# JiaxuanYou/graph-pooling

Hardware: AMD Instinct MI355X
Metric: graphs/sec fwd+bwd, DD padded batch N_max=500 (higher is better)
Workload: dtype f32; 1 GPU; S-DD: DD-shaped padded batch, B=20/GPU, N_max=500, F=89, H=E=20, K=50, L=3, 1 pool; graphs_per_gpu=20, global_batch=20, linkpred=False, hip_graph=True, parallelism=dp1

## Files before the change

graph_pooling_amd/csrc/dp_common.h:

```cpp
#pragma once
#include <hip/hip_runtime.h>
#include <cstddef>
#include <cstdint>
#include <cstdio>
#include <cstring>
#include <atomic>
#include <mutex>

#include "../../include/diffpool_hip.h"

namespace dp {

void set_error(const char* fmt, ...);
const char* last_error();

#define DP_CHECK_ARG(cond, ...)                      \
    do {                                             \
        if (!(cond)) {                               \
            ::dp::set_error(__VA_ARGS__);            \
            return DP_ERR_INVALID_ARG;               \
        }                                            \
    } while (0)

int* device_error_word();
int* level0_verdict_block();
int device_error_take(bool clear);
int device_error_gate(const char* entry);
#ifdef __HIPCC__
__device__ inline void dev_err_raise(int* word, int bit) {
    if (word) __hip_atomic_fetch_or(word, bit, __ATOMIC_RELAXED, __HIP_MEMORY_SCOPE_SYSTEM);
}

typedef unsigned int u32x4 __attribute__((ext_vector_type(4)));
struct ScBuf {
    __amdgpu_buffer_rsrc_t r;
};
__device__ __forceinline__ ScBuf sc_buf(const void* p, size_t bytes) {
    return ScBuf{__builtin_amdgcn_make_buffer_rsrc(const_cast<void*>(p), 0, (int)bytes, 0x00020000)};
}
__device__ __forceinline__ u32x4 sc_ld16(ScBuf b, unsigned off) { return __builtin_amdgcn_raw_buffer_load_b128(b.r, off, 0, 16); }
__device__ __forceinline__ void sc_st16(ScBuf b, unsigned off, u32x4 v) { __builtin_amdgcn_raw_buffer_store_b128(v, b.r, off, 0, 16); }
__device__ __forceinline__ float sc_ldf(ScBuf b, unsigned off) {
    return __uint_as_float(__builtin_amdgcn_raw_buffer_load_b32(b.r, off, 0, 16));
}
__device__ __forceinline__ void sc_stf(ScBuf b, unsigned off, float v) {
    __builtin_amdgcn_raw_buffer_store_b32(__float_as_uint(v), b.r, off, 0, 16);
}
__device__ __forceinline__ u32x4 sc_tagged(float v0, float v1, unsigned tag) {
    return (u32x4){__float_as_uint(v0), tag, __float_as_uint(v1), tag};
}
#endif

#ifdef __HIPCC__
__device__ __forceinline__ void lds_barrier() {
    asm volatile("" ::: "memory");
    __builtin_amdgcn_s_waitcnt(0xc07f);
    __builtin_amdgcn_s_barrier();
    asm volatile("" ::: "memory");
}
#endif

#ifdef __HIPCC__
template <int CTRL, int ROW_MASK, bool BOUND>
__device__ __forceinline__ float dpp_src(float old, float v) {
    return __int_as_float(__builtin_amdgcn_update_dpp(__float_as_int(old), __float_as_int(v), CTRL, ROW_MASK, 0xF, BOUND));
}
__device__ __forceinline__ float row16_sum(float v) {
    v += dpp_src<0xB1, 0xF, true>(0.f, v);
    v += dpp_src<0x4E, 0xF, true>(0.f, v);
    v += dpp_src<0x141, 0xF, true>(0.f, v);
    v += dpp_src<0x140, 0xF, true>(0.f, v);
    return v;
}
__device__ __forceinline__ float quad4_sum(float v) {
    v += dpp_src<0xB1, 0xF, true>(0.f, v);
    v += dpp_src<0x4E, 0xF, true>(0.f, v);
    return v;
}
__device__ __forceinline__ float oct8_sum(float v) {
    v = quad4_sum(v);
    v += dpp_src<0x141, 0xF, true>(0.f, v);
    return v;
}
__device__ __forceinline__ float row16_max(float v) {
    v = fmaxf(v, dpp_src<0xB1, 0xF, true>(v, v));
    v = fmaxf(v, dpp_src<0x4E, 0xF, true>(v, v));
    v = fmaxf(v, dpp_src<0x141, 0xF, true>(v, v));
    v = fmaxf(v, dpp_src<0x140, 0xF, true>(v, v));
    return v;
}
__device__ __forceinline__ float wave64_sum(float v) {
    v = row16_sum(v);
    v += dpp_src<0x142, 0xA, false>(0.f, v);
    v += dpp_src<0x143, 0xC, false>(0.f, v);
    return __int_as_float(__builtin_amdgcn_readlane(__float_as_int(v), 63));
}
__device__ __forceinline__ float wave64_max(float v) {
    v = row16_max(v);
    v = fmaxf(v, dpp_src<0x142, 0xA, false>(v, v));
    v = fmaxf(v, dpp_src<0x143, 0xC, false>(v, v));
    return __int_as_float(__builtin_amdgcn_readlane(__float_as_int(v), 63));
}
#endif

struct Seq {
    hipStream_t stream;
    char* ws;
    size_t ws_bytes;
    size_t ws_off;
    int err;
    bool dry;
    const int* pred = nullptr;
    void* fold_zero_p = nullptr;
    int fold_zero_n16 = 0;
    int* seq_word = nullptr;

    Seq(hipStream_t s, void* w, size_t wb) : stream(s), ws((char*)w), ws_bytes(wb), ws_off(0), err(0), dry(false) {}
    static Seq sizing() {
        Seq q(nullptr, nullptr, ~size_t(0) >> 1);
        q.dry = true;
        return q;
    }

    template <typename T>
    T* alloc(size_t n) {
        size_t bytes = (n * sizeof(T) + 255) & ~size_t(255);
        if (ws_off + bytes > ws_bytes) {
            if (!err) {
                set_error("workspace too small: need >= %zu bytes, have %zu", ws_off + bytes, ws_bytes);
                err = DP_ERR_WORKSPACE;
            }
            return nullptr;
        }
        T* p = (T*)(ws + ws_off);
        ws_off += bytes;
        return p;
    }
    bool ok() const { return err == 0 && !dry; }
    void copy(void* dst, const void* src, size_t bytes) {
        if (err || dry || bytes == 0) return;
        hipError_t e = hipMemcpyAsync(dst, src, bytes, hipMemcpyDeviceToDevice, stream);
        if (e != hipSuccess) {
            set_error("hipMemcpyAsync: %s", hipGetErrorString(e));
            err = (int)e;
        }
    }
    void check_launch(const char* what) {
        if (err) return;
        hipError_t e = hipGetLastError();
        if (e != hipSuccess) {
            set_error("%s: %s", what, hipGetErrorString(e));
            err = (int)e;
        }
    }
};

inline size_t align256(size_t b) { return (b + 255) & ~size_t(255); }

struct Knobs {
    int agg_wide;
    int agg_rt;
    int agg_debug;
    bool no_pack;
    bool gemm_trace;
    long gemm_target_wgs;
    int node_ksplit;
    bool no_head_fusion;
    bool no_level_fusion;
    bool no_head_fold;
    bool no_split_gemm;
    bool split_gemm_w4;
    bool no_row_quads;
    bool no_rowpart_hook;
    bool no_widen_fusion;
    bool no_agg_first;
    bool no_l0_persist_bwd;
    bool no_l0_persist;
    bool test_barrier_fail;
};
const Knobs& knobs();

struct DynLdsOnce {
    std::atomic<unsigned long long> done{0};
    std::mutex m;
};
void ensure_dyn_lds(Seq& q, DynLdsOnce& st, const void* fn, int bytes, const char* what);

void bgemm(Seq& q, const float* A, const float* B, float* C, const float* bias, int batch, int M, int N,
           int K, int lda, int ldb, int ldc, long sA, long sB, long sC, bool tA, bool tB, float alpha,
           float beta, int act);

#define GEMM_GROUP_MAX 4
struct GemmDesc {
    const float* A;
    const float* B;
    float* C;
    const float* bias;
    int M, N, K;
    int lda, ldb, ldc;
    long sA, sB, sC;
    bool tA, tB;
    float alpha, beta;
    int act;
    long sK;
    int atomic;
    unsigned short* split_out;
    int split_ct, split_k8, split_c0;
    int nosplit;
    float* fix_part;
    int* fix_cnt;
    const float* rp_xhat;
    int rp_ldx;
    float* rp_part;
    int rp_G, rp_g;
};
inline bool gemm_rowpart_ok(int N) { return N >= 1 && N <= 32; }
inline size_t gemm_fix_counters(int batch, int M, int N) {
    return (size_t)batch * ((M + 15) / 16) * ((N + 15) / 16);
}

__device__ inline void bf16_split3(float v, unsigned short& h, unsigned short& m, unsigned short& l) {
    auto rn = [](float x) -> unsigned {
        unsigned u = __float_as_uint(x);
        u += 0x7FFFu + ((u >> 16) & 1u);
        return u >> 16;
    };
    const unsigned hh = rn(v);
    const float r1 = v - __uint_as_float(hh << 16);
    const unsigned mm = rn(r1);
    const float r2 = r1 - __uint_as_float(mm << 16);
    h = (unsigned short)hh;
    m = (unsigned short)mm;
    l = (unsigned short)rn(r2);
}
__device__ __host__ inline long vs_index(int plane, int CTt, int K8, int cb, int k8, int c, int j) {
    return ((((long)plane * CTt + cb) * K8 + k8) * 16 + c) * 8 + j;
}
void bgemm_group(Seq& q, const GemmDesc* d, int count, int batch, int ksplit = 1);
struct GemmPick {
    int bm, bn;
    int ranges[GEMM_GROUP_MAX];
};
GemmPick gemm_pick(const GemmDesc* d, int count, int batch, int ksplit, bool hooked, long target);
long gemm_target_wgs();
int bgemm_plan(const GemmDesc* d, int count, int batch, int ksplit, int* plan_out);
bool gemm_split_usable(const GemmDesc& d, int batch, int ksplit);
void gemm_split_bf16(Seq& q, const GemmDesc& d, int batch);

struct RowGroups {
    int G;
    int c0[2];
    int w[2];
};
struct GroupPtrs {
    float* p[2];
    int ld[2];
};
struct GroupCPtrs {
    const float* p[2];
    int ld[2];
};

struct RowPick {
    int kernel;
    int nk;
    int quad;
    int finalize;
    int zero;
    bool generic() const { return kernel == DP_ROWK_SOFTMAX_FWD || kernel == DP_ROWK_SOFTMAX_BWD; }
};
RowPick rownorm_fwd_pick(const RowGroups& g);
RowPick rownorm_bwd_pick(const RowGroups& g, bool has_bn, int Bs);
RowPick bn_apply_fwd_pick(const RowGroups& g, bool has_part, int Bs);
RowPick softmax_mask_fwd_pick(int K, bool vs, bool zero, bool zero_aligned);
RowPick softmax_mask_bwd_pick(int K, bool dbias);
RowPick masked_max_fwd_pick(int n);
void rownorm_fwd(Seq& q, const float* U, int ldu, const float* P , GroupCPtrs bias,
                 RowGroups g, GroupPtrs yout, float* invn, float* part , long rows,
                 int normalize, int relu_stats);
void bn_apply_fwd(Seq& q, const float* Y, int ldy, const float* part , float* stats,
                  RowGroups g, GroupPtrs xout, int B, int n, int relu, int Bs = 0);
bool bn_transform_supported(RowGroups gin, RowGroups gout, int B);
void bn_transform_fwd(Seq& q, const float* Y, int ldy, const float* part, float* stats, RowGroups gin, GroupPtrs xout,
                      const float* const W[2], RowGroups gout, float* P, int ldp, int B, int n, int relu,
                      unsigned short* vs );
void mask_rows(Seq& q, const float* src, int lds, float* dst, int ldd, const int* num_nodes, int B, int n, int F);
void bn_bwd_partials(Seq& q, GroupCPtrs dx, GroupCPtrs xhat, RowGroups g, float* part, long rows);
void rownorm_bwd(Seq& q, GroupCPtrs dx, GroupCPtrs xhat , GroupCPtrs y,
                 const float* invn, const float* stats, const float* part2, RowGroups g, float* dU, int ldu,
                 const GroupPtrs* dbias , int B, int n, int has_relu, int has_bn,
                 int normalize, unsigned short* vs = nullptr ,
                 int Bs = 0 );
int rownorm_bwd_chunks(int n);
void colsum_batched(Seq& q, const float* X, int ldx, long strideX, int rows, int cols, float* out,
                    long strideOut, int batch, int rowsplit = 1, bool add = false );
void softmax_mask_fwd(Seq& q, const float* logits, int ldl, float* S, int lds, const int* num_nodes, int B,
                      int n, int K, float* S2 = nullptr, unsigned short* vs = nullptr, void* zero_p = nullptr,
                      size_t zero_bytes = 0);
void softmax_mask_bwd(Seq& q, const float* S, int lds, const float* dS, int ldds, const int* num_nodes,
                      float* dlogits, int ldl, int B, int n, int K, float* dbias = nullptr, long dbias_stride = 0,
                      const float* dS2 = nullptr );
void masked_max_fwd(Seq& q, const float* Z, int ldz, const int* num_nodes, float* out, int ldo, int* argmax,
                    int lda, int B, int n, int F);
void masked_max_bwd(Seq& q, const float* dout, int ldo, const int* argmax, int lda, float* dZ, int ldz, int B,
                    int n, int F);
void relu_bwd_inplace(Seq& q, float* d, const float* h, long count);
void argmax_rows(Seq& q, const float* X, int ldx, long long* out, int rows, int cols);
void ce_fwd(Seq& q, const float* logits, const long long* label, float* loss, float* prob, int B, int C,
            float* also_zero = nullptr ,
            float* dunit = nullptr );
void ce_bwd(Seq& q, const float* prob, const long long* label, const float* dloss, float scale, float* dlogits,
            int B, int C);
void reduce_slabs(Seq& q, const float* slabs, long stride, int B, float* out, long count, int accumulate);
void axpy(Seq& q, float* y, const float* x, float a, long count);
void mask_mul(Seq& q, const float* x, int ldx, const float* m, float* out, long rows, int w);
void mask_axpy(Seq& q, float* dst, int ldd, const float* src, const float* m, long rows, int w);
bool rownorm_bwd_mv_supported(RowGroups g, const int din[2], int n);
void rownorm_bwd_mv(Seq& q, GroupCPtrs dx, GroupCPtrs xhat, GroupCPtrs y, const float* invn, const float* stats,
                    const float* part2, RowGroups g, float* dU, int ldu, const GroupPtrs* dbias, int B, int n,
                    int has_relu, int has_bn, int normalize, int Bs, const float* const W[2], const int din[2],
                    const int c0in[2], float* dUin, int lddu);
bool widen_fwd_supported(RowGroups g, const int din[2]);
void widen_fwd(Seq& q, const float* Uin, int ldin, const int c0in[2], const int din[2], const float* const W[2],
               GroupCPtrs bias, RowGroups g, GroupPtrs yout, float* invn, long rows, int normalize);
void gather_cols(Seq& q, const float* x0, int ld0, int w0, const float* x1, int ld1, int w1, float* out, long rows);
bool scatter_add_cols_part_supported(int w0, int w1);
void scatter_add_cols_part(Seq& q, const float* src, GroupPtrs d, GroupCPtrs xhat, int w0, int w1, int G, float* part,
                           long rows);
void scatter_add_cols(Seq& q, const float* src, float* d0, int ld0, int w0, float* d1, int ld1, int w1, long rows);
void zero_fill(Seq& q, void* p, size_t bytes);
void zero_small(Seq& q, void* p, size_t bytes);

struct PackedAdj {
    const unsigned short* A;
    const unsigned short* At;
    int ld;
    const int* flag;
};
void adj_pack(Seq& q, const float* A, unsigned short* P, unsigned short* Pt, int* flag, int B, int n, int ld,
              bool flag_zeroed = false, void* zero_p = nullptr, size_t zero_bytes = 0);
int adj_pack_ld(int n);
bool adj_pack_supported(int n, int C);
size_t split3_elems(int B, int n, int C);
void aggregate(Seq& q, const float* A, const float* V, int ldv, float* U, int ldu, int B, int n, int C, bool trans,
               float beta, const PackedAdj* pk = nullptr, unsigned short* vs = nullptr, bool vs_ready = false);
bool aggregate_rownorm_fwd(Seq& q, const float* A, const float* V, int ldv, const float* P, GroupCPtrs bias,
                           RowGroups g, GroupPtrs yout, float* invn, float* part, int B, int n, int normalize,
                           int stats_mode, const PackedAdj* pk = nullptr, unsigned short* vs = nullptr,
                           bool vs_ready = false);
bool aggregate_packed_usable(const float* A, int n, int C);
struct AggPick {
    int form;
    int ct;
    int rt;
    int tiles, grid;
    size_t lds;
    int fallback;
    int fb_ct, fb_rt, fb_tiles, fb_grid;
    size_t fb_lds;
    bool packed;
    bool declines;
// ... 227 lines not shown
```

graph_pooling_amd/csrc/dp_head.hip:

```cpp
#include "dp_common.h"

namespace dp {

#ifdef DP_STAMP
__device__ unsigned long long g_head_stamps[16];
#define HEAD_STAMP(i)                                                                                 \
    do {                                                                                              \
        if (blockIdx.x == 0 && threadIdx.x == 0) g_head_stamps[i] = __builtin_amdgcn_s_memtime();     \
    } while (0)
#else
#define HEAD_STAMP(i) \
    do {              \
    } while (0)
#endif

constexpr int HEAD_FWD_LDS_FLOATS = 30 * 1024;
constexpr int HEAD_BWD_LDS_FLOATS = 38 * 1024;

__device__ inline float head_wave_sum(float v) {
    return wave64_sum(v);
}

template <int NT>
__device__ inline void head_stage(float* dst, const float* src, int cnt) {
    for (int e0 = 0; e0 < cnt; e0 += NT * 16) {
        float t[16];
#pragma unroll
        for (int u = 0; u < 16; ++u) t[u] = src[min(e0 + u * NT + (int)threadIdx.x, cnt - 1)];
#pragma unroll
        for (int u = 0; u < 16; ++u) {
            const int i = e0 + u * NT + (int)threadIdx.x;
            if (i < cnt) dst[i] = t[u];
        }
    }
}

template <int NT, typename Idx>
__device__ __forceinline__ void stage_issue(float (&t)[16], const float* src, int cnt, int e0, Idx idx) {
#pragma unroll
    for (int u = 0; u < 16; ++u) {
        if (e0 + u * NT >= cnt) break;
        t[u] = src[idx(min(e0 + u * NT + (int)threadIdx.x, cnt - 1))];
    }
}
template <int NT>
__device__ __forceinline__ void stage_commit(float* dst, const float (&t)[16], int cnt, int e0) {
#pragma unroll
    for (int u = 0; u < 16; ++u) {
        if (e0 + u * NT >= cnt) break;
        const int i = e0 + u * NT + (int)threadIdx.x;
        if (i < cnt) dst[i] = t[u];
    }
}
template <int NT, typename Idx>
__device__ inline void stage_rest(float* dst, const float* src, int cnt, Idx idx) {
    for (int e0 = NT * 16; e0 < cnt; e0 += NT * 16) {
        float t[16];
        stage_issue<NT>(t, src, cnt, e0, idx);
        stage_commit<NT>(dst, t, cnt, e0);
    }
}

struct HeadSizes {
    int wtot, btot, mx, hsum;
};
__host__ __device__ inline HeadSizes head_sizes(const HeadArgs& a) {
    HeadSizes z{0, 0, 0, 0};
    for (int i = 0; i < a.n_pred; ++i) {
        z.wtot += a.dims[i] * a.dims[i + 1];
        z.btot += a.dims[i + 1];
    }
    for (int i = 0; i <= a.n_pred; ++i) {
        z.mx = a.dims[i] > z.mx ? a.dims[i] : z.mx;
        z.hsum += a.dims[i];
    }
    return z;
}


__global__ __launch_bounds__(256) void k_head_fwd(HeadArgs a) {
    extern __shared__ float lds[];
    const HeadSizes z = head_sizes(a);
    float* Wl = lds;
    float* bl = Wl + z.wtot;
    float* h0 = bl + z.btot;
    float* h1 = h0 + z.mx;
    float* sv = h1 + z.mx;
    int* si = reinterpret_cast<int*>(sv + 256);
    const int b = blockIdx.x;
    const int lane = threadIdx.x & 63, wave = threadIdx.x >> 6;
    float* feat = a.hid[0] + (long)b * a.dims[0];
    HEAD_STAMP(0);
    constexpr int RU = 16;
    float zv[RU];
    const bool one_pass = a.Z && a.rw <= 64 && a.n <= 4 * RU;
    if (one_pass) {
        const float* zc = a.Z + (long)b * a.n * a.ldz + min(lane, a.rw - 1);
#pragma unroll
        for (int u = 0; u < RU; ++u) zv[u] = zc[(long)min(wave + 4 * u, a.n - 1) * a.ldz];
    }
    {
        const auto ident = [](int e) { return e; };
        float tf[16], tw[16], tb[16];
        stage_issue<256>(tf, feat, a.dims[0], 0, ident);
        int wo = 0, bo = 0;
        {
            const int cnt0 = a.dims[0] * a.dims[1];
            stage_issue<256>(tw, a.params + a.w_off[0], cnt0, 0, ident);
        }
        for (int i = 0; i < a.n_pred; ++i) {
            const int cnt = a.dims[i] * a.dims[i + 1], bc = a.dims[i + 1];
            const float* W = a.params + a.w_off[i];
            const float* bsrc = a.b_off[i] >= 0 ? a.params + a.b_off[i] : W;
            stage_issue<256>(tb, bsrc, bc, 0, ident);
            float tn[16];
            const bool more = i + 1 < a.n_pred;
            if (more) stage_issue<256>(tn, a.params + a.w_off[i + 1], a.dims[i + 1] * a.dims[i + 2], 0, ident);
            stage_commit<256>(Wl + wo, tw, cnt, 0);
            if (a.b_off[i] < 0) {
#pragma unroll
                for (int u = 0; u < 16; ++u) tb[u] = 0.f;
            }
            stage_commit<256>(bl + bo, tb, bc, 0);
            stage_rest<256>(Wl + wo, W, cnt, ident);
            if (a.b_off[i] >= 0) stage_rest<256>(bl + bo, bsrc, bc, ident);
            else
                for (int e = 4096 + threadIdx.x; e < bc; e += 256) bl[bo + e] = 0.f;
            if (more) {
#pragma unroll
                for (int u = 0; u < 16; ++u) tw[u] = tn[u];
            }
            wo += cnt;
            bo += bc;
        }
#pragma unroll
        for (int u = 0; u < 16; ++u) {
            const int k = u * 256 + (int)threadIdx.x;
            if (k < a.dims[0] && (!a.Z || k < a.featoff || k >= a.featoff + a.rw)) h0[k] = tf[u];
        }
        for (int k = 4096 + threadIdx.x; k < a.dims[0]; k += 256)
            if (!a.Z || k < a.featoff || k >= a.featoff + a.rw) h0[k] = feat[k];
    }
    HEAD_STAMP(1);
    if (a.Z) {
        for (int c0 = 0; c0 < a.rw; c0 += 64) {
            const int c = c0 + lane;
            float best = -INFINITY;
            int bi = -1;
            if (one_pass) {
#pragma unroll
                for (int u = 0; u < RU; ++u) {
                    const int r = wave + 4 * u;
                    if (r < a.n && zv[u] > best) {
                        best = zv[u];
                        bi = r;
                    }
                }
            } else if (c < a.rw) {
                const float* zc = a.Z + (long)b * a.n * a.ldz + c;
#pragma unroll 4
                for (int r = wave; r < a.n; r += 4) {
                    const float v = zc[(long)r * a.ldz];
                    if (v > best) {
                        best = v;
                        bi = r;
                    }
                }
            }
            sv[wave * 64 + lane] = best;
            si[wave * 64 + lane] = bi;
            __syncthreads();
            if (wave == 0 && c < a.rw) {
                for (int k = 1; k < 4; ++k) {
                    const float v = sv[k * 64 + lane];
                    const int i2 = si[k * 64 + lane];
                    if (i2 >= 0 && (v > best || (v == best && i2 < bi))) {
                        best = v;
                        bi = i2;
                    }
                }
                h0[a.featoff + c] = best;
                feat[a.featoff + c] = best;
                a.argmax[(long)b * a.lda + c] = bi;
            }
            __syncthreads();
        }
    }
    __syncthreads();
    HEAD_STAMP(2);
    float* cur = h0;
    float* nxt = h1;
    int wo = 0, bo = 0;
    bool poisoned = false;
    for (int i = 0; i < a.n_poison; ++i)
        poisoned |= __hip_atomic_load(a.poison[i], __ATOMIC_RELAXED, __HIP_MEMORY_SCOPE_AGENT) != 0;
    for (int i = 0; i < a.n_pred; ++i) {
        const int din = a.dims[i], dout = a.dims[i + 1];
        const bool last = i == a.n_pred - 1;
        float* out = a.hid[i + 1] + (long)b * dout;
        for (int j0 = 0; j0 < dout; j0 += 64) {
            const int j = j0 + lane;
            const int kq = (din + 3) / 4, kb = wave * kq, ke = min(din, kb + kq);
            float s = 0.f;
            if (j < dout) {
                const float* w = Wl + wo + j * din;
#pragma unroll 8
                for (int k = kb; k < ke; ++k) s += cur[k] * w[k];
            }
            sv[wave * 64 + lane] = s;
            __syncthreads();
            if (wave == 0 && j < dout) {
                s = sv[lane] + sv[64 + lane] + sv[128 + lane] + sv[192 + lane] + bl[bo + j];
                if (!last) s = fmaxf(s, 0.f);
                else if (poisoned) s = __builtin_nanf("");
                nxt[j] = s;
                out[j] = s;
            }
            __syncthreads();
        }
        __syncthreads();
        float* t = cur; cur = nxt; nxt = t;
        wo += din * dout;
        bo += dout;
    }
    if (a.labels && threadIdx.x == 0) {
        const int C = a.dims[a.n_pred];
        int best = 0;
        for (int c = 1; c < C; ++c)
            if (cur[c] > cur[best]) best = c;
        a.labels[b] = best;
    }
    HEAD_STAMP(3);
}

static size_t head_fwd_lds_floats(const HeadArgs& a) {
    const HeadSizes z = head_sizes(a);
    return (size_t)z.wtot + z.btot + 2 * z.mx + 512;
}
void head_fwd(Seq& q, const HeadArgs& a) {
    if (!q.ok()) return;
    static DynLdsOnce attr;
    ensure_dyn_lds(q, attr, reinterpret_cast<const void*>(&k_head_fwd), HEAD_FWD_LDS_FLOATS * (int)sizeof(float),
                   "k_head_fwd");
    if (!q.ok()) return;
    hipLaunchKernelGGL(k_head_fwd, dim3(a.B), dim3(256), head_fwd_lds_floats(a) * sizeof(float), q.stream, a);
    q.check_launch("head_fwd");
}

constexpr int HEAD_SLICE = 16;
__global__ __launch_bounds__(256) void k_head_bwd(HeadBwdArgs a) {
    extern __shared__ float lds[];
    const int B = a.h.B, L = a.h.n_pred;
    const int d0 = a.h.dims[0], d1 = a.h.dims[1];
    const int k0 = blockIdx.x * HEAD_SLICE, ks = min(HEAD_SLICE, d0 - k0);
    int wup = 0, hup = 0, mx = 0;
    for (int i = 1; i < L; ++i) {
        wup += a.h.dims[i] * a.h.dims[i + 1];
        hup += a.h.dims[i];
    }
    for (int i = 1; i <= L; ++i) mx = max(mx, a.h.dims[i]);
    float* Wu = lds;
    float* Hu = Wu + wup;
    float* W0 = Hu + (long)B * hup;
    float* F0 = W0 + d1 * HEAD_SLICE;
    float* g0 = F0 + B * HEAD_SLICE;
    float* g1 = g0 + (long)B * mx;
    HEAD_STAMP(8);
    int win[2] = {-1, -1};
#pragma unroll
    for (int it = 0; it < 2; ++it) {
        const int e = min((int)threadIdx.x + 256 * it, B * ks - 1);
        const int b = e / ks, k = k0 + e % ks;
        if (a.n_levels > 0) {
            const int* src = a.lv[0].argmax;
            for (int lv = 0; lv < a.n_levels; ++lv) {
                const int f = k - a.lv[lv].featoff;
                if (f >= 0 && f < a.lv[lv].rw) src = a.lv[lv].argmax + (long)b * a.lv[lv].lda + f;
            }
            win[it] = *src;
        }
    }
    {
        const auto ident = [](int e) { return e; };
        const auto slice = [=](int e) { return (long)(e >> 4) * d0 + k0 + min(e & 15, ks - 1); };
        static_assert(HEAD_SLICE == 16, "slice index math");
        const float* W0g = a.h.params + a.h.w_off[0];
        const float* F0g = a.h.hid[0];
        const int cW0 = d1 * HEAD_SLICE, cF0 = B * HEAD_SLICE, cG = B * a.h.dims[L];
        float tw0[16], tf0[16], tg[16];
        stage_issue<256>(tw0, W0g, cW0, 0, slice);
        stage_issue<256>(tf0, F0g, cF0, 0, slice);
        stage_issue<256>(tg, a.d_ypred, cG, 0, ident);
        int wo = 0, ho = 0;
        for (int i = 1; i < L; ++i) {
            const int cnt = a.h.dims[i] * a.h.dims[i + 1], hc = B * a.h.dims[i];
            const float* W = a.h.params + a.h.w_off[i];
            float tw[16], th[16];
            stage_issue<256>(tw, W, cnt, 0, ident);
            stage_issue<256>(th, a.h.hid[i], hc, 0, ident);
            stage_commit<256>(Wu + wo, tw, cnt, 0);
            stage_commit<256>(Hu + ho, th, hc, 0);
            stage_rest<256>(Wu + wo, W, cnt, ident);
            stage_rest<256>(Hu + ho, a.h.hid[i], hc, ident);
            wo += cnt;
            ho += hc;
        }
        stage_commit<256>(W0, tw0, cW0, 0);
        stage_commit<256>(F0, tf0, cF0, 0);
        stage_commit<256>(g0, tg, cG, 0);
        stage_rest<256>(W0, W0g, cW0, slice);
        stage_rest<256>(F0, F0g, cF0, slice);
        stage_rest<256>(g0, a.d_ypred, cG, ident);
    }
    __syncthreads();
    HEAD_STAMP(9);
    float* go = g0;
    float* gi = g1;
    int wo = wup, ho = B * hup;
    for (int i = L - 1; i >= 1; --i) {
        const int din = a.h.dims[i], dout = a.h.dims[i + 1];
        wo -= din * dout;
        ho -= B * din;
        const float* W = Wu + wo;
        const float* hin = Hu + ho;
        if (blockIdx.x == 0) {
            float* dW = a.grads + a.h.w_off[i];
            for (int e = threadIdx.x; e < dout * din; e += 256) {
                const int j = e / din, k = e % din;
                float s = 0.f;
#pragma unroll 8
                for (int b = 0; b < B; ++b) s += go[b * dout + j] * hin[b * din + k];
                dW[e] = s;
            }
            if (a.h.b_off[i] >= 0)
                for (int j = threadIdx.x; j < dout; j += 256) {
                    double s = 0.0;
#pragma unroll 8
                    for (int b = 0; b < B; ++b) s += (double)go[b * dout + j];
                    a.grads[a.h.b_off[i] + j] = (float)s;
                }
        }
        for (int e = threadIdx.x; e < B * din; e += 256) {
            const int b = e / din, k = e % din;
            float s = 0.f;
#pragma unroll 8
            for (int j = 0; j < dout; ++j) s += go[b * dout + j] * W[j * din + k];
            gi[e] = hin[e] > 0.f ? s : 0.f;
        }
        __syncthreads();
        float* t = go; go = gi; gi = t;
    }
    HEAD_STAMP(10);
    float* dW = a.grads + a.h.w_off[0];
    for (int e = threadIdx.x; e < d1 * ks; e += 256) {
        const int j = e / ks, kk = e % ks;
        float s = 0.f;
#pragma unroll 8
        for (int b = 0; b < B; ++b) s += go[b * d1 + j] * F0[b * HEAD_SLICE + kk];
        dW[(long)j * d0 + k0 + kk] = s;
    }
    if (blockIdx.x == 0 && a.h.b_off[0] >= 0)
        for (int j = threadIdx.x; j < d1; j += 256) {
            double s = 0.0;
#pragma unroll 8
            for (int b = 0; b < B; ++b) s += (double)go[b * d1 + j];
            a.grads[a.h.b_off[0] + j] = (float)s;
        }
    HEAD_STAMP(11);
    for (int e = threadIdx.x, it = 0; e < B * ks; e += 256, ++it) {
        const int b = e / ks, kk = e % ks, k = k0 + kk;
        float s = 0.f;
#pragma unroll 8
        for (int j = 0; j < d1; ++j) s += go[b * d1 + j] * W0[j * HEAD_SLICE + kk];
        for (int lv = 0; lv < a.n_levels; ++lv) {
            const HeadBwdArgs::Level& t = a.lv[lv];
            const int f = k - t.featoff;
            if (f >= 0 && f < t.rw) {
                const int r = it == 0 ? win[0] : it == 1 ? win[1] : t.argmax[(long)b * t.lda + f];
                if (r >= 0) t.dZ[((long)b * t.n + r) * t.ldz + f] = s;
            }
        }
    }
    HEAD_STAMP(12);
}

static size_t head_bwd_lds_floats(const HeadArgs& a) {
    size_t wup = 0, hup = 0, mx = 0;
    for (int i = 1; i < a.n_pred; ++i) {
        wup += (size_t)a.dims[i] * a.dims[i + 1];
        hup += a.dims[i];
    }
    for (int i = 1; i <= a.n_pred; ++i) mx = (size_t)a.dims[i] > mx ? a.dims[i] : mx;
    return wup + (size_t)a.B * hup + (size_t)a.dims[1] * HEAD_SLICE + (size_t)a.B * HEAD_SLICE + 2 * (size_t)a.B * mx;
}

bool head_supported(const HeadArgs& a) {
    if (a.n_pred < 1 || a.B < 1 || a.B > 1024) return false;
    return head_fwd_lds_floats(a) <= HEAD_FWD_LDS_FLOATS && head_bwd_lds_floats(a) <= HEAD_BWD_LDS_FLOATS;
}

void head_bwd(Seq& q, const HeadBwdArgs& a) {
    if (!q.ok()) return;
    static DynLdsOnce attr;
    ensure_dyn_lds(q, attr, reinterpret_cast<const void*>(&k_head_bwd), HEAD_BWD_LDS_FLOATS * (int)sizeof(float),
                   "k_head_bwd");
    if (!q.ok()) return;
    const int slices = (a.h.dims[0] + HEAD_SLICE - 1) / HEAD_SLICE;
    hipLaunchKernelGGL(k_head_bwd, dim3(slices), dim3(256), head_bwd_lds_floats(a.h) * sizeof(float), q.stream, a);
    q.check_launch("head_bwd");
}

#ifdef DP_STAMP
extern "C" __attribute__((visibility("default"))) int dp_debug_head_stamps(unsigned long long* out) {
    return (int)hipMemcpyFromSymbol(out, HIP_SYMBOL(g_head_stamps), sizeof(unsigned long long) * 16);
}
#endif

}
```

graph_pooling_amd/csrc/dp_small.hip:

```cpp
#include "dp_common.h"

namespace dp {

#define SM_L2_EPS 1e-12f
#define SM_BN_EPS 1e-5f

#ifdef DP_STAMP
__device__ unsigned long long g_small_stamps[2][32];
#define SM_STAMP(k, i)                                                                       \
    do {                                                                                     \
        if (blockIdx.x == 0 && threadIdx.x == 0) g_small_stamps[k][i] = __builtin_amdgcn_s_memtime(); \
    } while (0)
#else
#define SM_STAMP(k, i) \
    do {               \
    } while (0)
#endif

namespace {

__device__ inline float sm_team_sum(float v) {
    return row16_sum(v);
}

typedef float sm_f32x4 __attribute__((ext_vector_type(4)));

struct SmDiv {
    unsigned magic;
    int d;
    __device__ inline int quot(int e) const {
        return d == 1 ? e : (int)(((unsigned long long)(unsigned)e * magic) >> 32);
    }
    __device__ inline int rem(int e) const { return e - quot(e) * d; }
};
static SmDiv sm_div(int d) { return SmDiv{(unsigned)(0x100000000ull / (unsigned)d + 1), d}; }

template <typename SrcFn>
__device__ inline void sm_dma(float* dst, int count, SrcFn src_of) {
    const int lane = threadIdx.x & 63;
    const int wave = __builtin_amdgcn_readfirstlane(threadIdx.x >> 6), nw = blockDim.x >> 6;
    for (int c0 = wave * 64; c0 < count; c0 += nw * 64) {
        const int e = c0 + lane;
        if (e < count)
            __builtin_amdgcn_global_load_lds((const __attribute__((address_space(1))) void*)src_of(e),
                                             (__attribute__((address_space(3))) void*)(dst + c0), 4, 0, 0);
    }
}

template <bool TA, bool TB, typename Store>
__device__ inline void lds_mma(const float* A, int lda, const float* B, int ldb, int M, int N, int K, Store store,
                               int wave_shift = 0) {
    const int lane = threadIdx.x & 63, nwaves = blockDim.x >> 6;
    const int wave = ((threadIdx.x >> 6) + nwaves - wave_shift % nwaves) % nwaves;
    const int l15 = lane & 15, kq = lane >> 4;
    const int tm = (M + 15) / 16, tn = (N + 15) / 16;
    for (int t = wave; t < tm * tn; t += nwaves) {
        const int i = (t / tn) * 16 + l15, j = (t % tn) * 16 + l15;
        sm_f32x4 acc = (sm_f32x4){0.f, 0.f, 0.f, 0.f};
        const int ic = min(i, M - 1), jc = min(j, N - 1);
        const bool iok = i < M, jok = j < N;
#pragma unroll 8
        for (int k0 = 0; k0 < K; k0 += 4) {
            const int k = k0 + kq, kc = min(k, K - 1);
            const float ar = TA ? A[kc * lda + ic] : A[ic * lda + kc];
            const float br = TB ? B[jc * ldb + kc] : B[kc * ldb + jc];
            const float av = (k < K && iok) ? ar : 0.f;
            const float bv = (k < K && jok) ? br : 0.f;
            acc = __builtin_amdgcn_mfma_f32_16x16x4f32(av, bv, acc, 0, 0, 0);
        }
#pragma unroll
        for (int r = 0; r < 4; ++r) {
            const int row = (t / tn) * 16 + kq * 4 + r;
            if (row < M && j < N) store(row, j, acc[r]);
        }
    }
}


template <bool TA, bool TB, typename Store>
__device__ inline void lds_mma2(const float* A, int lda, const float* B, int ldb, int M, int N, int K, Store store,
                                int wave_shift = 0) {
    const int lane = threadIdx.x & 63, nwaves = blockDim.x >> 6;
    const int wave = ((threadIdx.x >> 6) + nwaves - wave_shift % nwaves) % nwaves;
    const int l15 = lane & 15, kq = lane >> 4;
    const int tm = (M + 15) / 16, tn = (N + 15) / 16;
    const int sa4 = 4 * (TA ? lda : 1), sb4 = 4 * (TB ? 1 : ldb);
    int tr = wave / tn, tc = wave - tr * tn;
    const int dr = nwaves / tn, dc = nwaves - dr * tn;
    for (; tr < tm; ) {
        const int i = tr * 16 + l15, j = tc * 16 + l15;
        const float* ap = (TA ? A + min(i, M - 1) : A + min(i, M - 1) * lda) + kq * (sa4 >> 2);
        const float* bp = (TB ? B + min(j, N - 1) * ldb : B + min(j, N - 1)) + kq * (sb4 >> 2);
        sm_f32x4 acc0 = (sm_f32x4){0.f, 0.f, 0.f, 0.f}, acc1 = acc0;
        int k = 0;
        for (; k + 16 <= K; k += 16) {
            const float a0 = ap[0], a1 = ap[sa4], a2 = ap[2 * sa4], a3 = ap[3 * sa4];
            const float b0 = bp[0], b1 = bp[sb4], b2 = bp[2 * sb4], b3 = bp[3 * sb4];
            ap += 4 * sa4;
            bp += 4 * sb4;
            acc0 = __builtin_amdgcn_mfma_f32_16x16x4f32(a0, b0, acc0, 0, 0, 0);
            acc1 = __builtin_amdgcn_mfma_f32_16x16x4f32(a1, b1, acc1, 0, 0, 0);
            acc0 = __builtin_amdgcn_mfma_f32_16x16x4f32(a2, b2, acc0, 0, 0, 0);
            acc1 = __builtin_amdgcn_mfma_f32_16x16x4f32(a3, b3, acc1, 0, 0, 0);
        }
        for (; k + 4 <= K; k += 4) {
            const float a0 = ap[0], b0 = bp[0];
            ap += sa4;
            bp += sb4;
            acc0 = __builtin_amdgcn_mfma_f32_16x16x4f32(a0, b0, acc0, 0, 0, 0);
        }
        if (k < K) {
            const bool kin = k + kq < K;
            const float a0 = ap[0], b0 = bp[0];
            acc1 = __builtin_amdgcn_mfma_f32_16x16x4f32(kin ? a0 : 0.f, kin ? b0 : 0.f, acc1, 0, 0, 0);
        }
#pragma unroll
        for (int r = 0; r < 4; ++r) {
            const int row = tr * 16 + kq * 4 + r;
            if (row < M && j < N) store(row, j, acc0[r] + acc1[r]);
        }
        tr += dr;
        tc += dc;
        if (tc >= tn) {
            tc -= tn;
            ++tr;
        }
    }
}

struct SmallFwdArgs {
    const float* adj;
    const float* x0;
    int ldx0;
    const float* yprev;
    int ldyp;
    const float* part_prev;
    float* stats_prev;
    float* xout;
    int ldxo;
    const float* W;
    const float* bias;
    float* y;
    int ldy;
    float* invn;
    float* part;
    int B, n, din, dout;
    int add_self, stats;
    SmDiv qdin;
};

__global__ __launch_bounds__(1024) void k_small_gcn_fwd(SmallFwdArgs a) {
    extern __shared__ __attribute__((aligned(16))) float lds[];
    const int b = blockIdx.x, tid = threadIdx.x;
    const int n = a.n, din = a.din, dout = a.dout;
    float* A = lds;
    float* X = A + n * n;
    float* W = X + n * din;
    float* P = W + din * dout;
    float* U = P + n * dout;
    float* mu = U + n * dout;
    float* rs = mu + n;
    float* BI = rs + n;
    float* PP = BI + dout;
    const int tl = tid & 15, team = tid >> 4;
    const int NT = blockDim.x, NTEAMS = blockDim.x >> 4;
    const bool bnprev = !a.x0 && a.part_prev;

    SM_STAMP(0, 0);
    sm_dma(A, n * n, [&](int e) { return a.adj + (long)b * n * n + e; });
    sm_dma(W, din * dout, [&](int e) { return a.W + e; });
    if (a.bias) sm_dma(BI, dout, [&](int e) { return a.bias + e; });
    else
        for (int i = tid; i < dout; i += NT) BI[i] = 0.f;
    {
        const float* xsrc = a.x0 ? a.x0 : a.yprev;
        const int ldx = a.x0 ? a.ldx0 : a.ldyp;
        sm_dma(X, n * din, [&](int e) { return xsrc + ((long)b * n + a.qdin.quot(e)) * ldx + a.qdin.rem(e); });
        if (bnprev) sm_dma(PP, a.B * n * 2, [&](int e) { return a.part_prev + e; });
    }
    __syncthreads();
    if (!a.x0) {
        for (int r = tid; r < n; r += NT) {
            float m = 0.f, rstd = 1.f;
            if (bnprev) {
                float sm = 0.f;
#pragma unroll 4
                for (int bb = 0; bb < a.B; ++bb) sm += PP[(bb * n + r) * 2];
                m = sm / (float)a.B;
                float s2 = 0.f;
#pragma unroll 4
                for (int bb = 0; bb < a.B; ++bb) {
                    const float d = PP[(bb * n + r) * 2] - m;
                    s2 += PP[(bb * n + r) * 2 + 1] + (float)din * d * d;
                }
                rstd = 1.0f / sqrtf(s2 / ((float)a.B * (float)din) + SM_BN_EPS);
                if (b == 0) {
                    a.stats_prev[r * 2] = m;
                    a.stats_prev[r * 2 + 1] = rstd;
                }
            }
            mu[r] = m;
            rs[r] = rstd;
        }
        __syncthreads();
        for (int r = team; r < n; r += NTEAMS)
            for (int k = tl; k < din; k += 16) {
                const float v = (fmaxf(X[r * din + k], 0.f) - mu[r]) * rs[r];
                X[r * din + k] = v;
                a.xout[((long)b * n + r) * a.ldxo + k] = v;
            }
        __syncthreads();
    }
    SM_STAMP(0, 1);
    lds_mma<false, false>(X, din, W, dout, n, dout, din, [&](int r, int c, float v) { P[r * dout + c] = v; });
    __syncthreads();
    SM_STAMP(0, 2);
    lds_mma<false, false>(A, n, P, dout, n, dout, n, [&](int r, int c, float v) {
        if (a.add_self) v += P[r * dout + c];
        U[r * dout + c] = v + BI[c];
    });
    __syncthreads();
    SM_STAMP(0, 3);
    for (int r = team; r < n; r += NTEAMS) {
        const long row = (long)b * n + r;
        float ss = 0.f;
        for (int c = tl; c < dout; c += 16) ss += U[r * dout + c] * U[r * dout + c];
        ss = sm_team_sum(ss);
        const float inv = 1.f / fmaxf(sqrtf(ss), SM_L2_EPS);
        float s1 = 0.f;
        for (int c = tl; c < dout; c += 16) {
            const float v = U[r * dout + c] * inv;
            a.y[row * a.ldy + c] = v;
            s1 += fmaxf(v, 0.f);
        }
        if (tl == 0) a.invn[row] = inv;
        if (a.stats) {
            s1 = sm_team_sum(s1);
            const float mean = s1 / (float)dout;
            float m2 = 0.f;
            for (int c = tl; c < dout; c += 16) {
                const float v = fmaxf(U[r * dout + c] * inv, 0.f) - mean;
                m2 += v * v;
            }
            m2 = sm_team_sum(m2);
            if (tl == 0) {
                a.part[row * 2] = mean;
                a.part[row * 2 + 1] = m2;
            }
        }
    }
    SM_STAMP(0, 4);
}

struct SmallBwdArgs {
    const float* adj;
    const float* xin;
    int ldxin;
    const float* W;
    const float* y;
    int ldy;
    const float* xhat;
    int ldxh;
    const float* invn;
    const float* stats;
    const float* part2;
    const float* dx;
    int lddx;
    float* dxin;
    int lddxin;
    float* part2_prev;
    float* dadj;
    float* dW;
    float* db;
    long slab_stride;
    int B, n, din, dout;
    int add_self, has_bn, has_relu;
    SmDiv qdin, qdout;
};

__global__ __launch_bounds__(1024) void k_small_gcn_bwd(SmallBwdArgs a) {
    extern __shared__ __attribute__((aligned(16))) float lds[];
    const int b = blockIdx.x, tid = threadIdx.x;
    const int n = a.n, din = a.din, dout = a.dout;
    float* A = lds;
    float* X = A + n * n;
    float* W = X + n * din;
    float* dU = W + din * dout;
    float* G = dU + n * dout;
    float* P = G + n * dout;
    float* XH = P + n * dout;
    float* DX = XH + n * dout;
    float* IV = DX + n * din;
    float* M0 = IV + n;
    float* M1 = M0 + n;
    float* DB = M1 + n;
    float* DBW = DB + dout;
    float* RS = DBW + 16 * dout;
    float* DA = RS + n;
    float* PP = DA + (a.dadj ? n * n : 0);
    const int tl = tid & 15, team = tid >> 4;
    const int NT = blockDim.x, NTEAMS = blockDim.x >> 4;
    float* dWb = a.dW + (long)b * a.slab_stride;
    float* dbb = a.db ? a.db + (long)b * a.slab_stride : nullptr;

    SM_STAMP(1, 0);
    sm_dma(A, n * n, [&](int e) { return a.adj + (long)b * n * n + e; });
    if (a.dadj) sm_dma(DA, n * n, [&](int e) { return a.dadj + (long)b * n * n + e; });
    if (a.has_bn) sm_dma(RS, n, [&](int e) { return a.stats + e * 2 + 1; });
    sm_dma(W, din * dout, [&](int e) { return a.W + e; });
    sm_dma(X, n * din, [&](int e) { return a.xin + ((long)b * n + a.qdin.quot(e)) * a.ldxin + a.qdin.rem(e); });
    if (a.dxin)
        sm_dma(DX, n * din, [&](int e) { return a.dxin + ((long)b * n + a.qdin.quot(e)) * a.lddxin + a.qdin.rem(e); });
    sm_dma(dU, n * dout, [&](int e) { return a.dx + ((long)b * n + a.qdout.quot(e)) * a.lddx + a.qdout.rem(e); });
    sm_dma(P, n * dout, [&](int e) { return a.y + ((long)b * n + a.qdout.quot(e)) * a.ldy + a.qdout.rem(e); });
    if (a.has_bn)
        sm_dma(XH, n * dout, [&](int e) { return a.xhat + ((long)b * n + a.qdout.quot(e)) * a.ldxh + a.qdout.rem(e); });
    sm_dma(IV, n, [&](int e) { return a.invn + (long)b * n + e; });
    if (a.has_bn) sm_dma(PP, a.B * n * 2, [&](int e) { return a.part2 + e; });
    for (int i = tid; i < 17 * dout; i += NT) DB[i] = 0.f;
    SM_STAMP(1, 8);
    __syncthreads();
    SM_STAMP(1, 9);
    if (a.has_bn) {
        for (int r = tid; r < n; r += NT) {
            float s0 = 0.f, s1 = 0.f;
#pragma unroll 4
            for (int bb = 0; bb < a.B; ++bb) {
                s0 += PP[(bb * n + r) * 2];
                s1 += PP[(bb * n + r) * 2 + 1];
            }
            const float cnt = (float)a.B * (float)dout;
            M0[r] = s0 / cnt;
            M1[r] = s1 / cnt;
        }
        __syncthreads();
    }
    SM_STAMP(1, 1);
    for (int r0 = 0; r0 < n; r0 += NTEAMS) {
        const int r = min(r0 + team, n - 1);
        const bool valid = r0 + team < n;
        const float rstd = a.has_bn ? RS[r] : 1.f;
        const float m0 = a.has_bn ? M0[r] : 0.f, m1 = a.has_bn ? M1[r] : 0.f;
        const float inv = IV[r];
        const bool project = inv < 1.0f / SM_L2_EPS;
        float dot = 0.f;
        for (int c = tl; c < dout; c += 16) {
            float d = dU[r * dout + c];
            const float yy = P[r * dout + c];
            if (a.has_bn) d = rstd * (d - m0 - XH[r * dout + c] * m1);
            if (a.has_relu) d = yy > 0.f ? d : 0.f;
// ... 775 lines not shown
```

Before: 86220 graphs/s.

## Rework head forward kernel: DMA staging, padded weights, 512 threads, split MLP groups

The head forward kernel now stages features, weights and biases into LDS with global_load_lds DMA, spread across waves with a rotating start wave, in place of register-staged copies. Weight rows can be padded by one float to avoid LDS bank conflicts. The block grows to 512 threads: four waves do the argmax readout while two groups of four waves compute separate output chunks of the MLP. Poison flags are loaded early, and lighter LDS barriers replace __syncthreads. This aims to cut load latency and sync overhead in a tiny per-graph kernel, at the cost of more complex indexing and host-side plan building.

New measurement: 87530 graphs/s, median of 6. 1.5% higher.

```diff
diff --git a/graph_pooling_amd/csrc/dp_common.h b/graph_pooling_amd/csrc/dp_common.h
--- a/graph_pooling_amd/csrc/dp_common.h
+++ b/graph_pooling_amd/csrc/dp_common.h
@@ -57,6 +57,36 @@
     __builtin_amdgcn_s_waitcnt(0xc07f);
     __builtin_amdgcn_s_barrier();
     asm volatile("" ::: "memory");
+}
+#endif
+
+#ifdef __HIPCC__
+__device__ __forceinline__ void sm_dma_piece(const float* src, float* lds_piece) {
+    __builtin_amdgcn_global_load_lds((const __attribute__((address_space(1))) void*)src,
+                                     (__attribute__((address_space(3))) void*)lds_piece, 4, 0, 0);
+}
+template <typename SrcFn>
+__device__ inline void sm_dma(float* dst, int count, SrcFn src_of, int first_wave = 0) {
+    const int lane = threadIdx.x & 63;
+    const int nw = blockDim.x >> 6;
+    int wave = __builtin_amdgcn_readfirstlane(threadIdx.x >> 6) - first_wave;
+    if (wave < 0) wave += nw;
+    for (int c0 = wave * 64; c0 < count; c0 += nw * 64) {
+        const int e = c0 + lane;
+        if (e < count) sm_dma_piece(src_of(e), dst + c0);
+    }
+}
+template <typename RowFn>
+__device__ inline void sm_dma_rows(float* dst, int ld, int rows, int len, RowFn row_src, int first_wave = 0) {
+    const int lane = threadIdx.x & 63;
+    const int nw = blockDim.x >> 6;
+    int wave = __builtin_amdgcn_readfirstlane(threadIdx.x >> 6) - first_wave;
+    if (wave < 0) wave += nw;
+    for (int r = wave; r < rows; r += nw) {
+        const float* src = row_src(r);
+        for (int c0 = 0; c0 < len; c0 += 64)
+            if (c0 + lane < len) sm_dma_piece(src + c0 + lane, dst + r * ld + c0);
+    }
 }
 #endif
 
diff --git a/graph_pooling_amd/csrc/dp_head.hip b/graph_pooling_amd/csrc/dp_head.hip
--- a/graph_pooling_amd/csrc/dp_head.hip
+++ b/graph_pooling_amd/csrc/dp_head.hip
@@ -16,23 +16,12 @@
 
 constexpr int HEAD_FWD_LDS_FLOATS = 30 * 1024;
 constexpr int HEAD_BWD_LDS_FLOATS = 38 * 1024;
+constexpr int HEAD_FWD_THREADS = 512;
+constexpr int HEAD_FWD_WAVES = HEAD_FWD_THREADS / 64;
+static_assert(HEAD_FWD_WAVES == 8, "k_head_fwd: four readout waves, two MLP groups of four, wave rotation by & 7");
 
 __device__ inline float head_wave_sum(float v) {
     return wave64_sum(v);
-}
-
-template <int NT>
-__device__ inline void head_stage(float* dst, const float* src, int cnt) {
-    for (int e0 = 0; e0 < cnt; e0 += NT * 16) {
-        float t[16];
-#pragma unroll
-        for (int u = 0; u < 16; ++u) t[u] = src[min(e0 + u * NT + (int)threadIdx.x, cnt - 1)];
-#pragma unroll
-        for (int u = 0; u < 16; ++u) {
-            const int i = e0 + u * NT + (int)threadIdx.x;
-            if (i < cnt) dst[i] = t[u];
-        }
-    }
 }
 
 template <int NT, typename Idx>
@@ -76,100 +65,129 @@
     }
     return z;
 }
-
-
-__global__ __launch_bounds__(256) void k_head_fwd(HeadArgs a) {
+constexpr int HEAD_PAD_MIN_DIN = 16;
+static int head_w_stride(int din, bool padded) {
+    return padded && !(din & 1) && din >= HEAD_PAD_MIN_DIN ? din + 1 : din;
+}
+struct alignas(32) HeadFwdLayer {
+    const float* W;
+    const float* bias;
+    float* out;
+    int din, dout;
+    int ws, wo;
+};
+struct HeadFwdArgs {
+    HeadFwdLayer L[DP_MAX_PRED + 1];
+    const float* Z;
+    int ldz, n, rw, featoff;
+    int* argmax;
+    int lda;
+    float* feat;
+    long long* labels;
+    const int* poison[DP_MAX_LEVELS + 1];
+    int n_poison;
+    int n_pred, d0, wtot, btot, mx;
+};
+
+
+__device__ __forceinline__ float head_dot(const float* x, const float* w, int n) {
+    float s = 0.f;
+    n = max(n, 0);
+    int k = 0;
+    for (; k < (n & 7); ++k) s = __builtin_fmaf(x[k], w[k], s);
+    {
+#pragma clang fp contract(off)
+        for (; k < n; k += 8) {
+#pragma unroll
+            for (int u = 0; u < 8; ++u) {
+                const float p = x[k + u] * w[k + u];
+                s = s + p;
+            }
+        }
+    }
+    return s;
+}
+
+__global__ __launch_bounds__(HEAD_FWD_THREADS) void k_head_fwd(HeadFwdArgs a) {
     extern __shared__ float lds[];
-    const HeadSizes z = head_sizes(a);
     float* Wl = lds;
-    float* bl = Wl + z.wtot;
-    float* h0 = bl + z.btot;
-    float* h1 = h0 + z.mx;
-    float* sv = h1 + z.mx;
+    float* bl = Wl + a.wtot;
+    float* h0 = bl + a.btot;
+    float* h1 = h0 + a.mx;
+    float* sv = h1 + a.mx;
     int* si = reinterpret_cast<int*>(sv + 256);
     const int b = blockIdx.x;
-    const int lane = threadIdx.x & 63, wave = threadIdx.x >> 6;
-    float* feat = a.hid[0] + (long)b * a.dims[0];
+    const int lane = threadIdx.x & 63, wave = __builtin_amdgcn_readfirstlane(threadIdx.x >> 6);
+    constexpr int nw = HEAD_FWD_WAVES;
+    float* feat = a.feat + (long)b * a.d0;
     HEAD_STAMP(0);
+    int pz[DP_MAX_LEVELS + 1];
+#pragma unroll
+    for (int i = 0; i < DP_MAX_LEVELS + 1; ++i) pz[i] = *a.poison[i];
     constexpr int RU = 16;
     float zv[RU];
     const bool one_pass = a.Z && a.rw <= 64 && a.n <= 4 * RU;
-    if (one_pass) {
+    if (one_pass && wave < 4) {
         const float* zc = a.Z + (long)b * a.n * a.ldz + min(lane, a.rw - 1);
 #pragma unroll
         for (int u = 0; u < RU; ++u) zv[u] = zc[(long)min(wave + 4 * u, a.n - 1) * a.ldz];
     }
     {
-        const auto ident = [](int e) { return e; };
-        float tf[16], tw[16], tb[16];
-        stage_issue<256>(tf, feat, a.dims[0], 0, ident);
-        int wo = 0, bo = 0;
-        {
-            const int cnt0 = a.dims[0] * a.dims[1];
-            stage_issue<256>(tw, a.params + a.w_off[0], cnt0, 0, ident);
-        }
+        int fw = 4 & (nw - 1);
+        const auto next = [&](int floats) { fw = (fw + ((floats + 63) >> 6)) & (nw - 1); };
+        sm_dma(h0, a.d0, [&](int e) { return feat + e; }, fw);
+        next(a.d0);
+        int bo = 0;
         for (int i = 0; i < a.n_pred; ++i) {
-            const int cnt = a.dims[i] * a.dims[i + 1], bc = a.dims[i + 1];
-            const float* W = a.params + a.w_off[i];
-            const float* bsrc = a.b_off[i] >= 0 ? a.params + a.b_off[i] : W;
-            stage_issue<256>(tb, bsrc, bc, 0, ident);
-            float tn[16];
-            const bool more = i + 1 < a.n_pred;
-            if (more) stage_issue<256>(tn, a.params + a.w_off[i + 1], a.dims[i + 1] * a.dims[i + 2], 0, ident);
-            stage_commit<256>(Wl + wo, tw, cnt, 0);
-            if (a.b_off[i] < 0) {
-#pragma unroll
-                for (int u = 0; u < 16; ++u) tb[u] = 0.f;
-            }
-            stage_commit<256>(bl + bo, tb, bc, 0);
-            stage_rest<256>(Wl + wo, W, cnt, ident);
-            if (a.b_off[i] >= 0) stage_rest<256>(bl + bo, bsrc, bc, ident);
-            else
-                for (int e = 4096 + threadIdx.x; e < bc; e += 256) bl[bo + e] = 0.f;
-            if (more) {
-#pragma unroll
-                for (int u = 0; u < 16; ++u) tw[u] = tn[u];
-            }
-            wo += cnt;
-            bo += bc;
-        }
-#pragma unroll
-        for (int u = 0; u < 16; ++u) {
-            const int k = u * 256 + (int)threadIdx.x;
-            if (k < a.dims[0] && (!a.Z || k < a.featoff || k >= a.featoff + a.rw)) h0[k] = tf[u];
-        }
-        for (int k = 4096 + threadIdx.x; k < a.dims[0]; k += 256)
-            if (!a.Z || k < a.featoff || k >= a.featoff + a.rw) h0[k] = feat[k];
-    }
-    HEAD_STAMP(1);
-    if (a.Z) {
+            const HeadFwdLayer l = a.L[i];
+            if (l.ws == l.din) {
+                sm_dma(Wl + l.wo, l.din * l.dout, [&](int e) { return l.W + e; }, fw);
+                next(l.din * l.dout);
+            } else {
+                sm_dma_rows(Wl + l.wo, l.ws, l.dout, l.din, [&](int r) { return l.W + (long)r * l.din; }, fw);
+                fw = (fw + l.dout) & (nw - 1);
+            }
+            if (l.bias) {
+                sm_dma(bl + bo, l.dout, [&](int e) { return l.bias + e; }, fw);
+                next(l.dout);
+            } else {
+                for (int e = threadIdx.x; e < l.dout; e += blockDim.x) bl[bo + e] = 0.f;
+            }
+            bo += l.dout;
+        }
+    }
+    HEAD_STAMP(4);
+    if (a.Z && a.rw > 0) {
         for (int c0 = 0; c0 < a.rw; c0 += 64) {
             const int c = c0 + lane;
             float best = -INFINITY;
             int bi = -1;
-            if (one_pass) {
-#pragma unroll
-                for (int u = 0; u < RU; ++u) {
-                    const int r = wave + 4 * u;
-                    if (r < a.n && zv[u] > best) {
-                        best = zv[u];
-                        bi = r;
+            if (wave < 4) {
+                if (one_pass) {
+#pragma unroll
+                    for (int u = 0; u < RU; ++u) {
+                        const int r = wave + 4 * u;
+                        if (r < a.n && zv[u] > best) {
+                            best = zv[u];
+                            bi = r;
+                        }
+                    }
+                } else if (c < a.rw) {
+                    const float* zc = a.Z + (long)b * a.n * a.ldz + c;
+#pragma unroll 4
+                    for (int r = wave; r < a.n; r += 4) {
+                        const float v = zc[(long)r * a.ldz];
+                        if (v > best) {
+                            best = v;
+                            bi = r;
+                        }
                     }
                 }
-            } else if (c < a.rw) {
-                const float* zc = a.Z + (long)b * a.n * a.ldz + c;
-#pragma unroll 4
-                for (int r = wave; r < a.n; r += 4) {
-                    const float v = zc[(long)r * a.ldz];
-                    if (v > best) {
-                        best = v;
-                        bi = r;
-                    }
-                }
-            }
-            sv[wave * 64 + lane] = best;
-            si[wave * 64 + lane] = bi;
+                sv[wave * 64 + lane] = best;
+                si[wave * 64 + lane] = bi;
+            }
             __syncthreads();
+            if (c0 == 0) HEAD_STAMP(1);
             if (wave == 0 && c < a.rw) {
                 for (int k = 1; k < 4; ++k) {
                     const float v = sv[k * 64 + lane];
@@ -183,48 +201,50 @@
                 feat[a.featoff + c] = best;
                 a.argmax[(long)b * a.lda + c] = bi;
             }
-            __syncthreads();
-        }
-    }
-    __syncthreads();
+            lds_barrier();
+        }
+    } else {
+        __syncthreads();
+        HEAD_STAMP(1);
+    }
     HEAD_STAMP(2);
     float* cur = h0;
     float* nxt = h1;
-    int wo = 0, bo = 0;
+    int bo = 0;
     bool poisoned = false;
-    for (int i = 0; i < a.n_poison; ++i)
-        poisoned |= __hip_atomic_load(a.poison[i], __ATOMIC_RELAXED, __HIP_MEMORY_SCOPE_AGENT) != 0;
+#pragma unroll
+    for (int i = 0; i < DP_MAX_LEVELS + 1; ++i) poisoned |= pz[i] != 0;
+    poisoned &= a.n_poison > 0;
+    const int grp = wave >> 2, kw = wave & 3;
+    constexpr int ngrp = 2;
+    float* sg = sv + grp * 256;
     for (int i = 0; i < a.n_pred; ++i) {
-        const int din = a.dims[i], dout = a.dims[i + 1];
+        const HeadFwdLayer l = a.L[i];
+        const int din = l.din, dout = l.dout, ws = l.ws, wo = l.wo;
         const bool last = i == a.n_pred - 1;
-        float* out = a.hid[i + 1] + (long)b * dout;
-        for (int j0 = 0; j0 < dout; j0 += 64) {
-            const int j = j0 + lane;
-            const int kq = (din + 3) / 4, kb = wave * kq, ke = min(din, kb + kq);
+        float* out = l.out + (long)b * dout;
+        for (int j0 = 0; j0 < dout; j0 += 64 * ngrp) {
+            const int j = j0 + grp * 64 + lane;
+            const bool mine = j < dout;
+            const int kq = (din + 3) / 4, kb = kw * kq, ke = min(din, kb + kq);
             float s = 0.f;
-            if (j < dout) {
-                const float* w = Wl + wo + j * din;
-#pragma unroll 8
-                for (int k = kb; k < ke; ++k) s += cur[k] * w[k];
-            }
-            sv[wave * 64 + lane] = s;
-            __syncthreads();
-            if (wave == 0 && j < dout) {
-                s = sv[lane] + sv[64 + lane] + sv[128 + lane] + sv[192 + lane] + bl[bo + j];
+            if (mine) s = head_dot(cur + kb, Wl + wo + j * ws + kb, ke - kb);
+            sg[kw * 64 + lane] = s;
+            lds_barrier();
+            if (kw == 0 && mine) {
+                s = sg[lane] + sg[64 + lane] + sg[128 + lane] + sg[192 + lane] + bl[bo + j];
                 if (!last) s = fmaxf(s, 0.f);
                 else if (poisoned) s = __builtin_nanf("");
                 nxt[j] = s;
                 out[j] = s;
             }
-            __syncthreads();
-        }
-        __syncthreads();
+            lds_barrier();
+        }
         float* t = cur; cur = nxt; nxt = t;
-        wo += din * dout;
         bo += dout;
     }
     if (a.labels && threadIdx.x == 0) {
-        const int C = a.dims[a.n_pred];
+        const int C = a.L[a.n_pred - 1].dout;
         int best = 0;
         for (int c = 1; c < C; ++c)
             if (cur[c] > cur[best]) best = c;
@@ -233,9 +253,39 @@
     HEAD_STAMP(3);
 }
 
-static size_t head_fwd_lds_floats(const HeadArgs& a) {
+static size_t head_fwd_lds_floats(const HeadArgs& a, bool padded) {
     const HeadSizes z = head_sizes(a);
-    return (size_t)z.wtot + z.btot + 2 * z.mx + 512;
+    size_t w = 0;
+    for (int i = 0; i < a.n_pred; ++i) w += (size_t)head_w_stride(a.dims[i], padded) * a.dims[i + 1];
+    return w + z.btot + 2 * z.mx + 512;
+}
+static bool head_fwd_padded(const HeadArgs& a) {
+    return head_fwd_lds_floats(a, true) <= (size_t)HEAD_FWD_LDS_FLOATS;
+}
+static HeadFwdArgs head_fwd_plan(const HeadArgs& a, bool padded) {
+    HeadFwdArgs k{};
+    const HeadSizes z = head_sizes(a);
+    int wo = 0;
+    for (int i = 0; i < a.n_pred; ++i) {
+        HeadFwdLayer& l = k.L[i];
+        l.W = a.params + a.w_off[i];
+        l.bias = a.b_off[i] >= 0 ? a.params + a.b_off[i] : nullptr;
+        l.out = a.hid[i + 1];
+        l.din = a.dims[i];
+        l.dout = a.dims[i + 1];
+        l.ws = head_w_stride(l.din, padded);
+        l.wo = wo;
+        wo += l.ws * l.dout;
+    }
+    k.Z = a.Z, k.ldz = a.ldz, k.n = a.n, k.rw = a.rw, k.featoff = a.featoff;
+    k.argmax = a.argmax, k.lda = a.lda;
+    k.feat = a.hid[0];
+    k.labels = a.labels;
+    for (int i = 0; i <= DP_MAX_LEVELS; ++i)
+        k.poison[i] = a.n_poison > 0 ? a.poison[i < a.n_poison ? i : 0] : reinterpret_cast<const int*>(a.params);
+    k.n_poison = a.n_poison;
+    k.n_pred = a.n_pred, k.d0 = a.dims[0], k.wtot = wo, k.btot = z.btot, k.mx = z.mx;
+    return k;
 }
 void head_fwd(Seq& q, const HeadArgs& a) {
     if (!q.ok()) return;
@@ -243,7 +293,9 @@
     ensure_dyn_lds(q, attr, reinterpret_cast<const void*>(&k_head_fwd), HEAD_FWD_LDS_FLOATS * (int)sizeof(float),
                    "k_head_fwd");
     if (!q.ok()) return;
-    hipLaunchKernelGGL(k_head_fwd, dim3(a.B), dim3(256), head_fwd_lds_floats(a) * sizeof(float), q.stream, a);
+    const bool padded = head_fwd_padded(a);
+    hipLaunchKernelGGL(k_head_fwd, dim3(a.B), dim3(HEAD_FWD_THREADS), head_fwd_lds_floats(a, padded) * sizeof(float),
+                       q.stream, head_fwd_plan(a, padded));
     q.check_launch("head_fwd");
 }
 
@@ -396,7 +448,7 @@
 
 bool head_supported(const HeadArgs& a) {
     if (a.n_pred < 1 || a.B < 1 || a.B > 1024) return false;
-    return head_fwd_lds_floats(a) <= HEAD_FWD_LDS_FLOATS && head_bwd_lds_floats(a) <= HEAD_BWD_LDS_FLOATS;
+    return head_fwd_lds_floats(a, false) <= HEAD_FWD_LDS_FLOATS && head_bwd_lds_floats(a) <= HEAD_BWD_LDS_FLOATS;
 }
 
 void head_bwd(Seq& q, const HeadBwdArgs& a) {
diff --git a/graph_pooling_amd/csrc/dp_small.hip b/graph_pooling_amd/csrc/dp_small.hip
--- a/graph_pooling_amd/csrc/dp_small.hip
+++ b/graph_pooling_amd/csrc/dp_small.hip
@@ -34,18 +34,6 @@
     __device__ inline int rem(int e) const { return e - quot(e) * d; }
 };
 static SmDiv sm_div(int d) { return SmDiv{(unsigned)(0x100000000ull / (unsigned)d + 1), d}; }
-
-template <typename SrcFn>
-__device__ inline void sm_dma(float* dst, int count, SrcFn src_of) {
-    const int lane = threadIdx.x & 63;
-    const int wave = __builtin_amdgcn_readfirstlane(threadIdx.x >> 6), nw = blockDim.x >> 6;
-    for (int c0 = wave * 64; c0 < count; c0 += nw * 64) {
-        const int e = c0 + lane;
-        if (e < count)
-            __builtin_amdgcn_global_load_lds((const __attribute__((address_space(1))) void*)src_of(e),
-                                             (__attribute__((address_space(3))) void*)(dst + c0), 4, 0, 0);
-    }
-}
 
 template <bool TA, bool TB, typename Store>
 __device__ inline void lds_mma(const float* A, int lda, const float* B, int ldb, int M, int N, int K, Store store,
```
